# lab-emi/CleanUMamba

Measured on AMD Instinct MI355X. Metric: audio samples/sec/node (train step, E8, 10s@16kHz), higher is better.
Workload: dtype f16

## Files before the change

cleanumamba_amd/csrc/gemm_tn.hip:

```cpp
#include "common.h"

namespace cum {

typedef __attribute__((ext_vector_type(8))) __bf16 bf16x8;
typedef __attribute__((ext_vector_type(4))) __bf16 bf16x4;
typedef __attribute__((ext_vector_type(8))) _Float16 f16x8;
typedef __attribute__((ext_vector_type(4))) _Float16 f16x4;
typedef __attribute__((ext_vector_type(4))) float f32x4;

struct TnParams {
  const void *dZ, *X;
  float *slab;
  float *bslab;
  int64_t ldz, ldx;
  int64_t M;
  int N, K;
  int Np, Kp;
  int rows_per_split, nsplit;
#ifdef CUM_AB
  int skip_store;
#endif
};

constexpr int TN_T = 128;

template <typename T>
struct TnCfg;
template <>
struct TnCfg<__bf16> {
  static constexpr int EPC = 8, BMK = 64;
  static __device__ __forceinline__ int swz(int row) { return 2 * ((row & 3) | (((row >> 3) & 1) << 2)); }
};
template <>
// ... 940 lines not shown
  if (tn_use8(M, N, K, dtype)) {
    *Np = N;
    *Kp = K;
    const int tiles = (N / 256) * (K / 256);
    int64_t want = tiles >= 256 ? 1 : 256 / tiles;
    if (force > 0) want = force;
    const int64_t max_s = (M + 255) / 256;
    if (want > max_s) want = max_s;
    int64_t rows = (M + want - 1) / want;
    rows = (rows + 63) / 64 * 64;
    *rps = (int)rows;
    *S = (int)((M + rows - 1) / rows);
    return;
  }
  *Np = (N + TN_T - 1) / TN_T * TN_T;
  *Kp = (K + TN_T - 1) / TN_T * TN_T;
  const int tiles = (*Np / TN_T) * (*Kp / TN_T);
  const int bmk = is16(dtype) ? 32 : 16;
  const int per_xcd = tiles >= 96 ? 1 : 96 / tiles;
  int64_t want = 8 * per_xcd;
  if (force > 0) want = force;
  const int64_t max_s = (M + 8 * bmk - 1) / (8 * bmk);
  if (want > max_s) want = max_s;
  if (want < 1) want = 1;
  int64_t rows = (M + want - 1) / want;
  rows = (rows + bmk - 1) / bmk * bmk;
  *rps = (int)rows;
  *S = (int)((M + rows - 1) / rows);
  if (*S < 1) *S = 1;
}

static int reduce_chunks(int S) { return S >= 64 ? 16 : 1; }

extern "C" int64_t cum_gemm_tn_workspace_elems(int32_t dtype, int64_t M, int32_t N, int32_t K) {
  int Np, Kp, S, rps;
  tn_plan(M, N, K, dtype, &Np, &Kp, &S, &rps);
  const int64_t C = reduce_chunks(S);
  return (int64_t)S * Np * Kp + (int64_t)S * Np + C * (int64_t)N * K + C * (int64_t)Np;
}

extern "C" int cum_gemm_tn_tile(int32_t dtype, int64_t M, int32_t N, int32_t K) {
  return tn_use8(M, N, K, dtype) ? 256 : tn_use_stream(M, N, K, dtype) ? 384 : TN_T;
}

extern "C" int cum_gemm_tn(int32_t dtype, int64_t M, int32_t N, int32_t K, const void *dZ, int64_t ldz, const void *X,
                           int64_t ldx, float *dW, int64_t ldw, float *db, float *workspace, void *stream) {
  CUM_REQUIRE(dtype_ok(dtype), "gemm_tn: dtype must be CUM_F32, CUM_BF16 or CUM_F16");
  CUM_REQUIRE(dZ && X && dW && workspace && M >= 0 && N > 0 && K > 0, "gemm_tn: bad argument");
  const int epc = is16(dtype) ? 8 : 4;
  CUM_REQUIRE(N % epc == 0 && K % epc == 0 && ldz % epc == 0 && ldx % epc == 0 && ldw % 4 == 0,
              "gemm_tn: N, K and strides must keep 16-byte alignment");
  CUM_REQUIRE(((uintptr_t)dZ & 15) == 0 && ((uintptr_t)X & 15) == 0 && ((uintptr_t)dW & 15) == 0,
              "gemm_tn: pointers must be 16-byte aligned");
  hipStream_t st = (hipStream_t)stream;
  const bool want_bias = db != nullptr;
  if (M == 0) {
    (void)hipMemset2DAsync(dW, sizeof(float) * ldw, 0, sizeof(float) * K, N, st);
    if (db) (void)hipMemsetAsync(db, 0, sizeof(float) * N, st);
    return CUM_OK;
  }
  int Np, Kp, S, rps;
  tn_plan(M, N, K, dtype, &Np, &Kp, &S, &rps);
  TnParams p{};
  p.dZ = dZ; p.X = X; p.ldz = ldz; p.ldx = ldx; p.M = M; p.N = N; p.K = K; p.Np = Np; p.Kp = Kp;
  p.rows_per_split = rps;
  p.nsplit = S;
// ... 6 lines not shown
  if (tn_use8(M, N, K, dtype)) {
    const int items = (N / 256) * (K / 256) * S;
    const dim3 grid8(8 * ((items + 7) / 8)), block8(512);
#ifdef CUM_AB
    if (cum_knob("CUM_TN9", 1) == 0) {
      if (dtype == CUM_BF16) hipLaunchKernelGGL(gemm_tn8_kernel<__bf16>, grid8, block8, 0, st, p);
      else hipLaunchKernelGGL(gemm_tn8_kernel<f16>, grid8, block8, 0, st, p);
    } else
#endif
    if (dtype == CUM_BF16)
      hipLaunchKernelGGL(gemm_tn9_kernel<__bf16>, grid8, block8, 0, st, p);
    else
      hipLaunchKernelGGL(gemm_tn9_kernel<f16>, grid8, block8, 0, st, p);
  } else if (tn_use_stream(M, N, K, dtype)) {
    CUM_REQUIRE((int64_t)rps * (ldz > ldx ? ldz : ldx) + 512 < (int64_t)1 << 31, "gemm_tn: a row split exceeds 2^31 elements");
    const dim3 gs(S), bs(512);
    if (Np == 128) {
      if (dtype == CUM_BF16) hipLaunchKernelGGL((gemm_tn_stream_kernel<__bf16, 128, 256>), gs, bs, 0, st, p);
      else hipLaunchKernelGGL((gemm_tn_stream_kernel<f16, 128, 256>), gs, bs, 0, st, p);
    } else {
      if (dtype == CUM_BF16) hipLaunchKernelGGL((gemm_tn_stream_kernel<__bf16, 256, 128>), gs, bs, 0, st, p);
      else hipLaunchKernelGGL((gemm_tn_stream_kernel<f16, 256, 128>), gs, bs, 0, st, p);
    }
  } else if (dtype == CUM_BF16)
    hipLaunchKernelGGL(gemm_tn_kernel<__bf16>, grid, block, 0, st, p);
  else if (dtype == CUM_F16)
    hipLaunchKernelGGL(gemm_tn_kernel<f16>, grid, block, 0, st, p);
  else
    hipLaunchKernelGGL(gemm_tn_kernel<float>, grid, block, 0, st, p);
  CUM_CHECK_LAUNCH();
#ifdef CUM_AB
  if (cum_knob("CUM_TN_NOREDUCE", 0)) return CUM_OK;
#endif
  const int C = reduce_chunks(S);
  float *part = workspace + (int64_t)S * Np * Kp + (int64_t)S * Np;
  float *bpart = part + (int64_t)C * N * K;
  const int cols4 = K / 4, bc4 = N / 4;
  const int gx = (int)(((int64_t)N * cols4 + 63) / 64), bx = want_bias ? (bc4 + 63) / 64 : 0;
  if (C == 1) {
    const ReduceJob w{p.slab, dW, (int64_t)Np * Kp, 0, ldw, Kp, N, cols4};
    const ReduceJob bj{p.bslab, db, (int64_t)Np, 0, N, Np, 1, bc4};
    hipLaunchKernelGGL(tn_reduce_kernel, dim3(gx + bx, 1), dim3(256), 0, st, w, bj, gx, S);
  } else {
    const ReduceJob w1{p.slab, part, (int64_t)Np * Kp, (int64_t)N * K, (int64_t)K, Kp, N, cols4};
    const ReduceJob b1{p.bslab, bpart, (int64_t)Np, (int64_t)Np, (int64_t)Np, Np, 1, bc4};
    hipLaunchKernelGGL(tn_reduce_kernel, dim3(gx + bx, C), dim3(256), 0, st, w1, b1, gx, S);
    const ReduceJob w2{part, dW, (int64_t)N * K, 0, ldw, K, N, cols4};
    const ReduceJob b2{bpart, db, (int64_t)Np, 0, N, Np, 1, bc4};
    hipLaunchKernelGGL(tn_reduce_kernel, dim3(gx + bx, 1), dim3(256), 0, st, w2, b2, gx, C);
  }
  CUM_CHECK_LAUNCH();
  return CUM_OK;
}
```

cleanumamba_amd/hip.py:

```python
import ctypes
import os

import torch

_HERE = os.path.dirname(os.path.abspath(__file__))
LIB_PATH = os.environ.get("CUM_LIB") or os.path.join(_HERE, "libcleanumamba_hip.so")

c_i32, c_i64, c_f32p, c_vp = ctypes.c_int32, ctypes.c_int64, ctypes.c_void_p, ctypes.c_void_p


class ScanShape(ctypes.Structure):
    _fields_ = [("batch", c_i32), ("dim", c_i32), ("dstate", c_i32), ("len", c_i32),
                ("u_sb", c_i64), ("u_sd", c_i64), ("u_sl", c_i64),
                ("dt_sb", c_i64), ("dt_sd", c_i64), ("dt_sl", c_i64),
                ("z_sb", c_i64), ("z_sd", c_i64), ("z_sl", c_i64),
                ("o_sb", c_i64), ("o_sd", c_i64), ("o_sl", c_i64),
                ("B_sb", c_i64), ("B_sn", c_i64), ("B_sl", c_i64),
                ("C_sb", c_i64), ("C_sn", c_i64), ("C_sl", c_i64),
                ("delta_softplus", c_i32), ("io_dtype", c_i32)]


class ScanGradStrides(ctypes.Structure):
    _fields_ = [("du_sb", c_i64), ("du_sd", c_i64), ("du_sl", c_i64),
                ("dd_sb", c_i64), ("dd_sd", c_i64), ("dd_sl", c_i64),
# ... 78 lines not shown
    "cum_stft_loss_fwd": (c_i32, [_P, _P, c_i64, c_i64, c_i32, c_i64, _P, _P, _P]),
    "cum_stft_loss_bwd": (c_i32, [_P, _P, c_i64, c_i64, c_i32, c_i64, _P, _P, _P, _P, _P]),
    "cum_stft_fold": (c_i32, [_P, c_i64, c_i64, c_i32, c_i32, c_i32, _P, c_i64, _P, c_i64, c_i32, _P]),
    "cum_gather": (c_i32, [c_i32, _P, _P, c_i64, c_i32, _P, _P]),
    "cum_pack2d": (c_i32, [_P, _P, _P, c_i32, _P, c_i32, _P, _P]),
    "cum_add_layernorm_fwd": (c_i32, [c_i32, c_i32, c_i64, c_i32, c_i32, _P, c_i64, c_i64, _P, _P, _P, ctypes.c_float,
                                      _P, _P, _P, _P, _P]),
    "cum_add_layernorm_bwd_workspace_elems": (c_i64, [c_i32]),
    "cum_add_layernorm_bwd": (c_i32, [c_i32, c_i32, c_i64, c_i32] + [_P] * 12),
    "cum_small_linear": (c_i32, [c_i32, c_i32, c_i32, _P, c_i64, _P, _P, _P, c_i64, _P]),
    "cum_mamba_step_supported": (c_i32, [c_i32] * 5),
    "cum_mamba_step": (c_i32, [c_i32] * 6 + [ctypes.c_float] + [_P] * 20),
    "cum_stream_window_update": (c_i32, [c_i32, c_i32, c_i32, c_i32, c_i32, _P, _P, c_i64, c_i64, c_i32, _P, _P, c_i64, _P]),
    "cum_stream_tail_rows": (c_i32, [c_i32, c_i32, c_i32, c_i32, _P, c_i64, c_i32, _P, c_i64, _P]),
    "cum_stream_overlap_add": (c_i32, [c_i32, c_i32, c_i32, c_i32, c_i32, _P, c_i64, _P, _P, _P, c_i64, _P, c_i64, c_i32, _P]),
    "cum_stream_hop_plan_ints": (c_i32, []),
    "cum_stream_hop_max_lds_bytes": (c_i32, []),
    "cum_stream_hop": (c_i32, [_P, _P, _P, c_i64, c_i32, _P, c_i64, _P, c_i64, c_i32, c_i32, _P]),
    "cum_stream_hop_slots": (c_i32, [_P, _P, _P, c_i64, c_i32, _P, _P, c_i32, _P, c_i64, _P, c_i64, c_i32, _P]),
    "cum_stream_pool_stage": (c_i32, [_P, c_i64, c_i32, _P, _P, c_i32, _P, c_i64, _P, c_i64, _P]),
    "cum_fft_plan_create": (c_i32, [c_i32, c_i32, c_i64, ctypes.POINTER(ctypes.c_void_p), ctypes.POINTER(c_i64)]),
    "cum_fft_plan_destroy": (c_i32, [_P]),
    "cum_fft_exec": (c_i32, [_P, _P, _P, c_i32, _P, _P]),
    "cum_stft_fused_supported": (c_i32, [c_i32]),
    "cum_stft_fused_workspace_elems": (c_i64, [c_i64, c_i64]),
    "cum_stft_fused_fwd": (c_i32, [_P, _P, c_i64, c_i64, c_i64, c_i64, c_i32, c_i32, c_i32, _P, _P, c_i64, c_i64, _P, _P, _P]),
    "cum_stft_fused_bwd": (c_i32, [_P, _P, c_i64, c_i64, c_i64, c_i64, c_i32, c_i32, c_i32, _P, _P, c_i64, c_i64, _P, _P, _P,
                                   _P, _P]),
    "cum_stft_loss_fwd_packed": (c_i32, [_P, _P, c_i64, c_i64, c_i32, c_i64, _P, _P, _P, _P]),
    "cum_stft_loss_bwd_packed": (c_i32, [_P, _P, c_i64, c_i64, c_i32, c_i64, _P, _P, _P, _P, _P, _P]),
    "cum_enc0_fwd": (c_i32, [c_i32, c_i64, c_i32, c_i32, _P, _P, _P, _P, _P, _P, c_i64, _P, _P]),
    "cum_ench_fwd": (c_i32, [c_i32, c_i64, c_i32, c_i32, _P, c_i64, _P, _P, _P, _P, _P, c_i64, _P, _P, c_i64, _P, _P]),
    "cum_dech_fwd": (c_i32, [c_i32, c_i64, c_i32, c_i32, _P, c_i64, _P, _P, _P, _P, _P, _P, c_i64, _P, _P, c_i64, _P, _P]),
    "cum_enc0_bwd_workgroups": (c_i32, [c_i64]),
    "cum_enc0_bwd_workspace_elems": (c_i64, [c_i64]),
    "cum_enc0_bwd": (c_i32, [c_i32, c_i64, c_i32, c_i32, _P, _P, _P, _P, _P, _P, _P, _P, _P]),
    "cum_dec7_fwd": (c_i32, [c_i32, c_i64, c_i32, c_i32, _P, _P, _P, _P, _P, _P, c_i64, _P]),
    "cum_dec7_bwd_workgroups": (c_i32, [c_i64]),
    "cum_dec7_bwd_workspace_elems": (c_i64, [c_i64]),
    "cum_dec7_bwd": (c_i32, [c_i32, c_i64, c_i32, c_i32, _P, _P, _P, _P, _P, _P, _P, _P, c_i64, _P, _P, _P, _P]),
    "cum_lp_loss_parts": (c_i32, [c_i64]),
    "cum_lp_loss_fwd": (c_i32, [c_i32, _P, _P, c_i64, _P, _P, _P]),
    "cum_lp_loss_bwd": (c_i32, [c_i32, _P, _P, c_i64, _P, _P, _P]),
    "cum_clip_std_parts": (c_i32, [c_i64]),
    "cum_clip_std": (c_i32, [_P, c_i32, c_i64, c_i64, ctypes.c_float, _P, _P, _P]),
    "cum_frame_rows": (c_i32, [c_i32, _P, c_i32, c_i64, c_i64, c_i64, c_i64, _P, c_i32, _P, _P]),
    "cum_unframe_rows": (c_i32, [c_i32, _P, c_i32, c_i64, c_i64, _P, _P, _P]),
    "cum_optim_state_elems": (c_i32, []),
    "cum_optim_sumsq_parts": (c_i32, [c_i64]),
    "cum_optim_sumsq": (c_i32, [_P, c_i64, _P, _P]),
    "cum_optim_prepare": (c_i32, [_P, _P, c_i32, ctypes.c_float, ctypes.c_double, ctypes.c_double, c_i32, ctypes.c_float,
                                  ctypes.c_float, c_i32, _P]),
    "cum_ssd_chunk": (c_i32, []),
    "cum_ssd_states_elems": (c_i64, [c_i32] * 5),
    "cum_ssd_bwd_workspace_elems": (c_i64, [c_i32] * 5),
    "cum_ssd_fwd": (c_i32, [ctypes.POINTER(SsdShape)] + [_P] * 11),
    "cum_ssd_bwd": (c_i32, [ctypes.POINTER(SsdShape)] + [_P] * 12 + [c_i64, c_i64, _P, c_i64, c_i64] + [_P] * 5),
    "cum_gated_rmsnorm_fwd": (c_i32, [c_i32, c_i64, c_i32, _P, c_i64, _P, c_i64, _P, ctypes.c_float, _P, c_i64, _P, _P]),
    "cum_gated_rmsnorm_bwd_workspace_elems": (c_i64, [c_i32]),
    "cum_gated_rmsnorm_bwd": (c_i32, [c_i32, c_i64, c_i32, _P, c_i64, _P, c_i64, _P, _P, _P, c_i64, _P, c_i64, _P, c_i64,
                                      _P, _P, _P]),
    "cum_ssd_step": (c_i32, [c_i32] * 5 + [ctypes.c_float, _P, c_i64] + [_P] * 9 + [c_i64, _P]),
    "cum_optim_adam": (c_i32, [_P, _P, _P, _P, c_i64, _P, ctypes.c_double, ctypes.c_double, ctypes.c_float, ctypes.c_float,
                               _P]),
    "cum_metrics_frame_count": (c_i64, [c_i64]),
    "cum_metrics_reduce_keep": (c_i64, [c_i64]),
# ... 121 lines not shown
```

cleanumamba_amd/network/convstack.py:

```python
import ctypes
import os

import numpy as np
import torch

from .. import hip


def rup(x, m):
    return (x + m - 1) // m * m


class Geo:

    def __init__(self, B, T, C):
        self.B, self.T, self.C = B, T, C
        self.P = T + 2
        self.Cp = rup(C, 8)
        self.M = B * self.P
        self.slack = 2 + (128 + self.Cp - 1) // self.Cp
        self.R = 1 + self.M + self.slack

    def new(self, dtype, device, zero=False):
        if zero:
# ... 1023 lines not shown
_DECH_FUSED = os.environ.get("CUM_DECH_FUSED", "1") != "0"


def _dech_ok(w1, wt, skip, relu, gi, gg, go, dt):
    return (_DECH_FUSED and _SIGN_MASK and relu and skip is not None and dt in hip.HALF_TYPES
            and tuple(w1.shape) == (256, 128, 1) and tuple(wt.shape) == (128, 64, 4)
            and gi.Cp == 128 and gg.Cp == 128 and go.Cp == 64 and gg.P >= 3)


def _dech_fwd(ubuf, w1, b1, wt, bt, skip, gi, gg, go, save_z):
    dt, dev = ubuf.dtype, ubuf.device
    sh1, sht = tuple(w1.shape), tuple(wt.shape)
    w1p = take(w1, ("glu_fwd", sh1, 256, 128), lambda: lay_glu_fwd(sh1, 256, 128), dt)
    b1p = take(b1, ("glu_vec", 256), lambda: lay_glu_vec(256), torch.float32)
    wtp = take(wt, ("convt_fwd", sht, gg.Cp, go.Cp, 128, 256), lambda: lay_convt_fwd(sht, gg.Cp, go.Cp, 128, 256), dt)

    def bias_layout():
        out = torch.zeros(128, dtype=torch.int64)
        out.view(2, 64)[:, :64] = _ids((64,))
        return out
    btp = take(bt, ("convt_vec", 64, go.Cp, 128), bias_layout, torch.float32)
    ybuf = go.new(dt, dev)
    g = gg.new(dt, dev) if save_z else None
    z = torch.empty(gg.M, 128, dtype=dt, device=dev) if save_z else None
    act = torch.empty(go.R * go.Cp // 4, dtype=torch.uint8, device=dev) if save_z else None
    with torch.cuda.device(dev):
        hip.check(hip.lib().cum_dech_fwd(
            hip.dtype_code(dt), gg.M, gg.P, gg.T, hip.ptr(ubuf), gi.R, hip.ptr(w1p), hip.ptr(b1p), hip.ptr(wtp),
            hip.ptr(btp), hip.ptr(skip[1:]), hip.ptr(g), gg.tail, hip.ptr(z), hip.ptr(ybuf[1:]), go.tail,
            hip.ptr(act[go.Cp // 4:]) if act is not None else None, hip.stream_ptr()))
    return g, z, ybuf, act


def _enc0_bwd(dz, xbuf, w1, b1, w2, gm, go, slot_w1, slot_w2):
    dt, dev = dz.dtype, dz.device
    wp = _enc0_w2p(w2, gm, dt)
    lib = hip.lib()
    ws = torch.empty(lib.cum_enc0_bwd_workspace_elems(go.M), dtype=torch.float32, device=dev)
    (a1, o1), (a2, o2) = slot_w1, slot_w2
    with torch.cuda.device(dev):
        hip.check(lib.cum_enc0_bwd(hip.dtype_code(dt), go.M, go.P, go.T, hip.ptr(dz), hip.ptr(xbuf), hip.ptr(w1.detach()),
                                   hip.ptr(b1.detach()), hip.ptr(wp), ctypes.c_void_p(a2.data_ptr() + 4 * o2),
                                   ctypes.c_void_p(a1.data_ptr() + 4 * o1), hip.ptr(ws), hip.stream_ptr()))


_DEC7_FUSED = os.environ.get("CUM_DEC7_FUSED", "1") != "0"


def _dec7_ok(w1, wt, gi, gg, go, dt):
    return (_DEC7_FUSED and dt in hip.HALF_TYPES and tuple(w1.shape) == (128, 64, 1) and tuple(wt.shape) == (64, 1, 4)
            and gi.C == 64 and gg.C == 64 and go.C == 1 and go.Cp == 8 and gi.P >= 32 and w1.dtype == torch.float32
            and wt.dtype == torch.float32)


def _dec7_fwd(ubuf, w1, b1, wt, bt, gi, go):
    dt, dev = ubuf.dtype, ubuf.device
    wp = _enc0_w2p(w1, gi, dt)
    bp = take(b1, ("glu_vec", w1.shape[0]), lambda: lay_glu_vec(w1.shape[0]), torch.float32)
    ybuf = go.new(dt, dev)
    with torch.cuda.device(dev):
        hip.check(hip.lib().cum_dec7_fwd(hip.dtype_code(dt), gi.M, gi.P, gi.T, hip.ptr(ubuf), hip.ptr(wp), hip.ptr(bp),
                                         hip.ptr(wt.detach()), hip.ptr(bt.detach()), hip.ptr(ybuf), go.tail, hip.stream_ptr()))
    return ybuf


def _dec7_bwd(dy, ubuf, mask_bits, w1, b1, wt, gi, slot_w1, slot_wt):
# ... 58 lines not shown
        def parts(lo, hi):
            out = []
            for i in range(lo, hi):
                gi, gm, _ = geos[i]
                sh1, sh2 = shapes[4 * i], shapes[4 * i + 2]
                G32 = 2 * zs[i].shape[1]
                out.append(arena.dw_index(2 * i, _invert(lay_conv_fwd(sh1, gi.Cp, gm.Cp, 4 * gi.Cp), sh1)))
                out.append(arena.db_index(2 * i, torch.arange(1, sh1[0] + 1, dtype=torch.int64)))
                out.append(arena.dw_index(2 * i + 1, _invert(lay_glu_fwd(sh2, G32, gm.Cp), sh2)))
                out.append(arena.db_index(2 * i + 1, _invert(lay_glu_vec(sh2[0]), (sh2[0],))))
            return out
        key = ("enc", tuple(shapes), tuple((g[0].Cp, g[1].Cp) for g in geos), tuple(z.shape[1] for z in zs))

        def deliver(lo, hi):
            grads[4 * lo:4 * hi] = arena.deliver((key, lo, hi), params[4 * lo:4 * hi], shapes[4 * lo:4 * hi],
                                                 lambda: parts(lo, hi))
        cut = E - 3 if E > 3 else 0
        sink = grad_sink(params) if cut > 0 else None
        early = sink is not None and getattr(sink[0], "early_announce", False)
        for i in reversed(range(E)):
            gi, gm, go = geos[i]
            w1, b1, w2, b2 = params[4 * i:4 * i + 4]
            if dz is None:
                if dys[i] is None:
                    raise RuntimeError("EncoderStack: the deepest output must be used")
                dz = _glu_bwd(zs[i], bufs[i + 1], dys[i].contiguous(), go)
            G32 = dz.shape[1]
            y1 = y1s[i]
            if y1 is None:
                if not ctx.needs_input_grad[0]:
                    _enc0_bwd(dz, bufs[0], w1, b1, w2, gm, go, arena.out(0), arena.out(1))
                    break
                y1 = _conv_relu_fwd(bufs[0], w1, b1, gi, gm)
            _glu_wgrad(dz, y1, gm, go.M, arena.out(2 * i + 1))
            wt = _glu_dgrad_weights(w2, gm, G32, dt)
            dzc = gm.new(dt, dev)
            if bits[i] is not None:
                gemm(dz, 0, G32, wt, None, dzc, gm.Cp, gm.Cp, gm.M, gm.P, gm.T, hip.EPI_MASK, gm.Cp,
                     res=bits[i][gm.Cp // 4:], r_off=0, ldr=gm.Cp, geo=gm, mask_bits=True)
            else:
                gemm(dz, 0, G32, wt, None, dzc, gm.Cp, gm.Cp, gm.M, gm.P, gm.T, hip.EPI_MASK, gm.Cp,
                     res=y1, r_off=gm.Cp, ldr=gm.Cp, geo=gm)
            sh = tuple(w1.shape)
            wgrad(dzc, gm.Cp, gm.Cp, gm.Cp, bufs[i], gi.Cp, 2 * gi.Cp, 4 * gi.Cp, gm.M, out=arena.out(2 * i))
            dz = None
            if early and i == cut:
                deliver(cut, E)
            if i == 0 and not ctx.needs_input_grad[0]:
                break
            Nd, Kd = rup(2 * gi.Cp, 16), rup(2 * gm.Cp, bk_of(dt))
            wd = take(w1, ("conv_dgrad", sh, gi.Cp, gm.Cp, Nd, Kd), lambda: lay_conv_dgrad(sh, gi.Cp, gm.Cp, Nd, Kd), dt)
            ext = None if i == 0 or dys[i - 1] is None else dys[i - 1].contiguous()
            if i > 0 and gi.Cp % 16 == 0:
                dz = torch.empty(gi.M, 2 * gi.Cp, dtype=dt, device=dev)
                gemm(dzc, 0, gm.Cp, wd, None, dz, 0, 4 * gi.Cp, gm.M, gm.P, gm.T + 1, hip.EPI_GLU_BWD, 2 * gi.Cp,
                     res=ext, r_off=gi.Cp, ldr=2 * gi.Cp, aux=zs[i - 1], x_off=0, ldz=2 * gi.Cp,
                     aux2=bufs[i], y_off=gi.Cp, ldy=2 * gi.Cp, gate_only=True)
                continue
            dx = gi.new(dt, dev)
            gemm(dzc, 0, gm.Cp, wd, None, dx, gi.Cp, 2 * gi.Cp, gm.M, gm.P, gm.T + 1, hip.EPI_BIAS, 2 * gi.Cp, geo=gi)
            if i == 0:
                dx0 = dx
            else:
                dz = _glu_bwd(zs[i - 1], bufs[i], dx if ext is None else dx + ext, gi)
        deliver(0, cut if early else E)
        return (dx0, None, None, *grads)


def _convt_bias_grad(bt, dbp, Cp, C, dtype):
    sink = grad_sink([bt]) if (bt.is_leaf and bt.dtype == torch.float32) else None
    if sink is not None:
        flat, idx, offs = sink
        torch.add(dbp[:C], dbp[Cp:Cp + C], out=flat.grad[offs[0]:offs[0] + C])
        flat.wrote(idx)
        return None
# ... 122 lines not shown
```

include/cleanumamba_hip.h:

```cpp
#ifndef CLEANUMAMBA_HIP_H
#define CLEANUMAMBA_HIP_H

#include <stdint.h>

#ifdef __cplusplus
extern "C" {
#endif

#define CUM_OK 0
#define CUM_EINVAL (-1)
#define CUM_ELAUNCH (-2)
#define CUM_EWORKSPACE (-3)

#define CUM_ABI_VERSION 16

int cum_abi_version(void);
const char *cum_last_error(void);

int cum_scan_chunk(void);

#define CUM_SCAN_SOFTPLUS 1
#define CUM_SCAN_A_IS_LOG 2
typedef struct {
  int32_t batch, dim, dstate, len;
// ... 183 lines not shown
int cum_stream_overlap_add(int32_t dtype, int32_t streams, int32_t L2, int32_t Cp, int32_t C, const void *y,
                           int64_t y_pitch, void *tail, const float *bias, const void *skip, int64_t skip_pitch,
                           void *out, int64_t out_pitch, int32_t relu, void *stream);

int cum_stream_hop_plan_ints(void);
int cum_stream_hop_max_lds_bytes(void);
int cum_stream_hop(const void *plan, const float *weights, float *state, int64_t state_stride, int32_t streams,
                   const float *in, int64_t in_stride, float *out, int64_t out_stride, int32_t n_hops,
                   int32_t lds_bytes, void *stream);

int cum_stream_hop_slots(const void *plan, const float *weights, float *state, int64_t state_stride, int32_t capacity,
                         const int32_t *items_host, const int32_t *items, int32_t n_items, const float *in,
                         int64_t in_stride, float *out, int64_t out_stride, int32_t lds_bytes, void *stream);
int cum_stream_pool_stage(float *hist, int64_t hist_stride, int32_t capacity, const int32_t *recs_host,
                          const int32_t *recs, int32_t n_recs, const float *x, int64_t x_stride, float *stage,
                          int64_t stage_stride, void *stream);

int cum_enc0_fwd(int32_t dtype, int64_t M, int32_t pitch, int32_t valid, const void *xin, const float *w1,
                 const float *b1, const void *w2p, const float *b2p, void *out, int64_t zero_tail, void *gate,
                 void *stream);
int32_t cum_enc0_bwd_workgroups(int64_t M);
int64_t cum_enc0_bwd_workspace_elems(int64_t M);
int cum_enc0_bwd(int32_t dtype, int64_t M, int32_t pitch, int32_t valid, const void *dZ, const void *xin,
                 const float *w1, const float *b1, const void *w2p, float *slot_w2, float *slot_w1, float *workspace,
                 void *stream);

int cum_ench_fwd(int32_t dtype, int64_t M, int32_t pitch, int32_t valid, const void *xin, int64_t x_rows,
                 const void *w1p, const float *b1p, const void *w2p, const float *b2p, void *y1, int64_t y1_tail,
                 void *bits, void *out, int64_t out_tail, void *gate, void *stream);

int cum_dech_fwd(int32_t dtype, int64_t M, int32_t pitch, int32_t valid, const void *u, int64_t u_rows,
                 const void *w1p, const float *b1p, const void *wtp, const float *btp, const void *skip, void *g,
                 int64_t g_tail, void *gate, void *out, int64_t out_tail, void *bits, void *stream);

int cum_dec7_fwd(int32_t dtype, int64_t M, int32_t pitch, int32_t valid, const void *u, const void *w1p, const float *b1p,
                 const float *wt, const float *bt, void *out, int64_t zero_tail, void *stream);
int32_t cum_dec7_bwd_workgroups(int64_t M);
int64_t cum_dec7_bwd_workspace_elems(int64_t M);
int cum_dec7_bwd(int32_t dtype, int64_t M, int32_t pitch, int32_t valid, const void *dY, const void *u, const void *mask,
                 const void *w1p, const float *b1p, const float *wt, void *dU, void *dpre, int64_t zero_tail,
                 float *slot_w1, float *slot_wt, float *workspace, void *stream);

int32_t cum_lp_loss_parts(int64_t n);
int cum_lp_loss_fwd(int32_t p, const float *y, const float *c, int64_t n, float *partials, float *out, void *stream);
int cum_lp_loss_bwd(int32_t p, const float *y, const float *c, int64_t n, const float *gout, float *dy, void *stream);

int32_t cum_clip_std_parts(int64_t len);
int cum_clip_std(const float *x, int32_t rows, int64_t len, int64_t stride, float eps, float *partials, float *out,
                 void *stream);

int cum_frame_rows(int32_t dtype, const float *x, int32_t batch, int64_t len, int64_t stride, int64_t T,
                   int64_t total_rows, const float *scale, int32_t invert, void *out, void *stream);
int cum_unframe_rows(int32_t dtype, const void *rows, int32_t batch, int64_t len, int64_t T, const float *scale,
                     float *y, void *stream);

int32_t cum_optim_state_elems(void);
int32_t cum_optim_sumsq_parts(int64_t n);
int cum_optim_sumsq(const float *g, int64_t n, float *partials, void *stream);
int cum_optim_prepare(float *state, const float *partials, int32_t nparts, float max_norm, double beta1, double beta2,
                      int32_t use_scaler, float growth, float backoff, int32_t growth_interval, void *stream);
int cum_optim_adam(float *p, const float *g, float *m, float *v, int64_t n, const float *state, double beta1,
                   double beta2, float eps, float weight_decay, void *stream);

typedef struct {
  int32_t batch, len, nheads, headdim, dstate;
  int64_t x_sb, x_sl, dt_sb, dt_sl, B_sb, B_sl, C_sb, C_sl, y_sb, y_sl;
// ... 80 lines not shown
```

Before: 130.8 million.

## Fuse GLU weight-grad and masked data-grad GEMMs into one pointwise pair backward kernel

Adds a HIP kernel that streams dZ and X tiles through LDS once and computes both the weight gradient (TN GEMM, with bias sum into per-split slabs) and the masked data gradient (dZ times W with sign-bit mask and valid-time zeroing) in the same pass. The slab reduction is factored out of gemm_tn so the new kernel can reuse it. The encoder backward path uses the new kernel for the 256x128 pointwise layer when mask bits exist. The goal is to avoid reading dZ twice and to save a launch, in exchange for a specialized, shape-restricted kernel with inline-asm wait counts.

```diff
diff --git a/cleanumamba_amd/csrc/gemm_tn.h b/cleanumamba_amd/csrc/gemm_tn.h
--- /dev/null
+++ b/cleanumamba_amd/csrc/gemm_tn.h
@@ -0,0 +1,10 @@
+#pragma once
+#include "common.h"
+
+namespace cum {
+
+int tn_reduce_chunks(int S);
+void tn_reduce_slabs(const float *slab, const float *bslab, float *part, int S, int N, int K, int Np, int Kp, float *dW,
+                     int64_t ldw, float *db, hipStream_t st);
+
+}
diff --git a/cleanumamba_amd/csrc/gemm_tn.hip b/cleanumamba_amd/csrc/gemm_tn.hip
--- a/cleanumamba_amd/csrc/gemm_tn.hip
+++ b/cleanumamba_amd/csrc/gemm_tn.hip
@@ -1,4 +1,5 @@
 #include "common.h"
+#include "gemm_tn.h"
 
 namespace cum {
 
@@ -1005,6 +1006,30 @@
 
 static int reduce_chunks(int S) { return S >= 64 ? 16 : 1; }
 
+namespace cum {
+int tn_reduce_chunks(int S) { return reduce_chunks(S); }
+void tn_reduce_slabs(const float *slab, const float *bslab, float *part, int S, int N, int K, int Np, int Kp, float *dW,
+                     int64_t ldw, float *db, hipStream_t st) {
+  const bool want_bias = bslab != nullptr;
+  const int C = reduce_chunks(S);
+  float *bpart = part + (int64_t)C * N * K;
+  const int cols4 = K / 4, bc4 = N / 4;
+  const int gx = (int)(((int64_t)N * cols4 + 63) / 64), bx = want_bias ? (bc4 + 63) / 64 : 0;
+  if (C == 1) {
+    const ReduceJob w{slab, dW, (int64_t)Np * Kp, 0, ldw, Kp, N, cols4};
+    const ReduceJob bj{bslab, db, (int64_t)Np, 0, N, Np, 1, bc4};
+    hipLaunchKernelGGL(tn_reduce_kernel, dim3(gx + bx, 1), dim3(256), 0, st, w, bj, gx, S);
+  } else {
+    const ReduceJob w1{slab, part, (int64_t)Np * Kp, (int64_t)N * K, (int64_t)K, Kp, N, cols4};
+    const ReduceJob b1{bslab, bpart, (int64_t)Np, (int64_t)Np, (int64_t)Np, Np, 1, bc4};
+    hipLaunchKernelGGL(tn_reduce_kernel, dim3(gx + bx, C), dim3(256), 0, st, w1, b1, gx, S);
+    const ReduceJob w2{part, dW, (int64_t)N * K, 0, ldw, K, N, cols4};
+    const ReduceJob b2{bpart, db, (int64_t)Np, 0, N, Np, 1, bc4};
+    hipLaunchKernelGGL(tn_reduce_kernel, dim3(gx + bx, 1), dim3(256), 0, st, w2, b2, gx, C);
+  }
+}
+}
+
 extern "C" int64_t cum_gemm_tn_workspace_elems(int32_t dtype, int64_t M, int32_t N, int32_t K) {
   int Np, Kp, S, rps;
   tn_plan(M, N, K, dtype, &Np, &Kp, &S, &rps);
@@ -1077,23 +1102,7 @@
 #ifdef CUM_AB
   if (cum_knob("CUM_TN_NOREDUCE", 0)) return CUM_OK;
 #endif
-  const int C = reduce_chunks(S);
-  float *part = workspace + (int64_t)S * Np * Kp + (int64_t)S * Np;
-  float *bpart = part + (int64_t)C * N * K;
-  const int cols4 = K / 4, bc4 = N / 4;
-  const int gx = (int)(((int64_t)N * cols4 + 63) / 64), bx = want_bias ? (bc4 + 63) / 64 : 0;
-  if (C == 1) {
-    const ReduceJob w{p.slab, dW, (int64_t)Np * Kp, 0, ldw, Kp, N, cols4};
-    const ReduceJob bj{p.bslab, db, (int64_t)Np, 0, N, Np, 1, bc4};
-    hipLaunchKernelGGL(tn_reduce_kernel, dim3(gx + bx, 1), dim3(256), 0, st, w, bj, gx, S);
-  } else {
-    const ReduceJob w1{p.slab, part, (int64_t)Np * Kp, (int64_t)N * K, (int64_t)K, Kp, N, cols4};
-    const ReduceJob b1{p.bslab, bpart, (int64_t)Np, (int64_t)Np, (int64_t)Np, Np, 1, bc4};
-    hipLaunchKernelGGL(tn_reduce_kernel, dim3(gx + bx, C), dim3(256), 0, st, w1, b1, gx, S);
-    const ReduceJob w2{part, dW, (int64_t)N * K, 0, ldw, K, N, cols4};
-    const ReduceJob b2{bpart, db, (int64_t)Np, 0, N, Np, 1, bc4};
-    hipLaunchKernelGGL(tn_reduce_kernel, dim3(gx + bx, 1), dim3(256), 0, st, w2, b2, gx, C);
-  }
+  tn_reduce_slabs(p.slab, p.bslab, workspace + (int64_t)S * Np * Kp + (int64_t)S * Np, S, N, K, Np, Kp, dW, ldw, db, st);
   CUM_CHECK_LAUNCH();
   return CUM_OK;
 }
diff --git a/cleanumamba_amd/csrc/pair_bwd.hip b/cleanumamba_amd/csrc/pair_bwd.hip
--- /dev/null
+++ b/cleanumamba_amd/csrc/pair_bwd.hip
@@ -0,0 +1,388 @@
+#include "common.h"
+#include "gemm_tn.h"
+
+namespace cum {
+
+typedef __attribute__((ext_vector_type(8))) __bf16 pw_bf16x8;
+typedef __attribute__((ext_vector_type(8))) _Float16 pw_f16x8;
+typedef __attribute__((ext_vector_type(4))) float pw_f32x4;
+typedef __attribute__((ext_vector_type(2))) unsigned pw_u32x2;
+typedef __attribute__((ext_vector_type(4))) unsigned pw_u32x4;
+
+struct PairParams {
+  const void *dZ, *X, *W;
+  const unsigned char *bits;
+  void *out, *aux;
+  float *slab, *bslab;
+  int64_t M, out_tail;
+  int rows_per_split, nsplit;
+  unsigned pitch, valid;
+};
+
+__device__ __forceinline__ int pw_swz(int row) { return 2 * ((row & 3) | (((row >> 3) & 1) << 2)); }
+
+template <typename T>
+__device__ __forceinline__ pw_f32x4 pw_mfma(pw_u32x4 a, pw_u32x4 b, pw_f32x4 c) {
+  if constexpr (__is_same(T, f16))
+    return __builtin_amdgcn_mfma_f32_16x16x32_f16(__builtin_bit_cast(pw_f16x8, a), __builtin_bit_cast(pw_f16x8, b), c, 0, 0, 0);
+  else
+    return __builtin_amdgcn_mfma_f32_16x16x32_bf16(__builtin_bit_cast(pw_bf16x8, a), __builtin_bit_cast(pw_bf16x8, b), c, 0, 0, 0);
+}
+
+template <typename T>
+__device__ __forceinline__ unsigned pw_pack2(float a, float b) {
+  typedef T V2 __attribute__((ext_vector_type(2)));
+  V2 v = {(T)a, (T)b};
+  return __builtin_bit_cast(unsigned, v);
+}
+
+template <typename T, bool AUX>
+__global__ __launch_bounds__(512) void pw_pair_bwd_kernel(const PairParams p) {
+  static_assert(sizeof(T) == 2, "16-bit element types only");
+  constexpr int NT = 256, KT = 128;
+  constexpr int EPC = 8, BMK = 64, NST = 3;
+  constexpr int CZ = NT / EPC, CX = KT / EPC;
+  constexpr int ZCH = BMK * CZ, XCH = BMK * CX;
+  constexpr int BCH = BMK * (KT / 4) / 16;
+  constexpr int NZ = ZCH / 512, NX = XCH / 512;
+  constexpr int NDMA = NZ + NX + 1;
+  constexpr int NSTORE = AUX ? 8 : 4;
+  constexpr int STG = ZCH + XCH + BCH;
+  constexpr int WN = NT / 64;
+  __shared__ uint4 lds[NST * STG];
+
+  const int tid = threadIdx.x, lane = tid & 63;
+  const int wave = uniform(tid >> 6);
+  const int wn = wave % WN, wk = wave / WN;
+  const int g = lane >> 4, r = lane & 15;
+  const int sp = blockIdx.x;
+  const int64_t m_begin = (int64_t)sp * p.rows_per_split;
+  int64_t m_end = m_begin + p.rows_per_split;
+  m_end = m_end < p.M ? m_end : p.M;
+  const int rows = (int)(m_end - m_begin);
+  const T *dZ = static_cast<const T *>(p.dZ) + m_begin * NT;
+  const T *X = static_cast<const T *>(p.X) + m_begin * KT;
+  const unsigned char *bits = p.bits ? p.bits + m_begin * (KT / 4) : nullptr;
+  T *out = static_cast<T *>(p.out) + m_begin * KT;
+  T *aux = AUX ? static_cast<T *>(p.aux) + m_begin * KT : nullptr;
+
+  typedef __attribute__((address_space(3))) void *lds_ptr;
+  typedef const __attribute__((address_space(1))) void *glb_ptr;
+
+  pw_u32x4 wf[8];
+  {
+    const T *W = static_cast<const T *>(p.W) + (16 * wave + r) * NT + 8 * g;
+#pragma unroll
+    for (int kb = 0; kb < 8; ++kb) wf[kb] = *reinterpret_cast<const pw_u32x4 *>(W + 32 * kb);
+    asm volatile("s_waitcnt vmcnt(0)"
+                 : "+v"(wf[0]), "+v"(wf[1]), "+v"(wf[2]), "+v"(wf[3]), "+v"(wf[4]), "+v"(wf[5]), "+v"(wf[6]), "+v"(wf[7])
+                 : : "memory");
+  }
+
+  int zrow[NZ], zoff[NZ], xrow[NX], xoff[NX];
+#pragma unroll
+  for (int i = 0; i < NZ; ++i) {
+    const int pos = i * 512 + tid;
+    zrow[i] = pos / CZ;
+    zoff[i] = ((pos % CZ) ^ pw_swz(zrow[i])) * EPC;
+  }
+#pragma unroll
+  for (int i = 0; i < NX; ++i) {
+    const int pos = i * 512 + tid;
+    xrow[i] = pos / CX;
+    xoff[i] = ((pos % CX) ^ pw_swz(xrow[i])) * EPC;
+  }
+  const int brow = tid >> 3, boff = (tid & 7) * 4;
+  auto issue = [&](int s, int buf) {
+    uint4 *st = lds + buf * STG;
+#pragma unroll
+    for (int i = 0; i < NZ; ++i) {
+      int m = s * BMK + zrow[i];
+      m = m < rows ? m : rows - 1;
+      __builtin_amdgcn_global_load_lds((glb_ptr)(dZ + (m * NT + zoff[i])), (lds_ptr)(&st[i * 512 + wave * 64]), 16, 0, 0);
+    }
+#pragma unroll
+    for (int i = 0; i < NX; ++i) {
+      int m = s * BMK + xrow[i];
+      m = m < rows ? m : rows - 1;
+      __builtin_amdgcn_global_load_lds((glb_ptr)(X + (m * KT + xoff[i])), (lds_ptr)(&st[ZCH + i * 512 + wave * 64]), 16, 0, 0);
+    }
+    {
+      int m = s * BMK + brow;
+      m = m < rows ? m : rows - 1;
+      const unsigned char *src = bits ? bits + (m * (KT / 4) + boff) : reinterpret_cast<const unsigned char *>(dZ + m * NT) + boff;
+      __builtin_amdgcn_global_load_lds((glb_ptr)src, (lds_ptr)(&st[ZCH + XCH + wave * 16]), 4, 0, 0);
+    }
+  };
+
+  constexpr int BROWS = 512 / CZ;
+  const int bc = tid % CZ;
+  float bsum[EPC];
+#pragma unroll
+  for (int e = 0; e < EPC; ++e) bsum[e] = 0.f;
+
+  pw_f32x4 acc[4][4];
+#pragma unroll
+  for (int i = 0; i < 4; ++i)
+#pragma unroll
+    for (int j = 0; j < 4; ++j) acc[i][j] = pw_f32x4{0.f, 0.f, 0.f, 0.f};
+
+  const unsigned lds0 = (unsigned)(uintptr_t)(lds_ptr)lds;
+  const int q = r >> 2, pp = r & 3;
+  const int r0 = 8 * g + q, s0 = pw_swz(r0);
+  unsigned ax[4], az[4], ab[BMK / BROWS], ad[4];
+#pragma unroll
+  for (int i = 0; i < 4; ++i) {
+    ax[i] = (unsigned)((ZCH + r0 * CX + ((wk * 8 + 2 * i) ^ s0)) * 16 + pp * 8);
+    az[i] = (unsigned)((r0 * CZ + ((wn * 8 + 2 * i) ^ s0)) * 16 + pp * 8);
+    ad[i] = (unsigned)((r * CZ + ((4 * i + g) ^ pw_swz(r))) * 16);
+  }
+#pragma unroll
+  for (int i = 0; i < BMK / BROWS; ++i) {
+    const int row = tid / CZ + BROWS * i;
+    ab[i] = (unsigned)((row * CZ + (bc ^ pw_swz(row))) * 16);
+  }
+  const unsigned am = (unsigned)((ZCH + XCH) * 16 + r * (KT / 4) + 4 * wave + g);
+#define CUM_TR(dst, addr, off) asm volatile("ds_read_b64_tr_b16 %0, %1 offset:%2" : "=v"(dst) : "v"(addr), "n"(off) : "memory")
+#define CUM_RD128(dst, addr, off) asm volatile("ds_read_b128 %0, %1 offset:%2" : "=v"(dst) : "v"(addr), "n"(off) : "memory")
+
+  unsigned t0 = (unsigned)(m_begin % p.pitch);
+  const int nsteps = (rows + BMK - 1) / BMK;
+  issue(0, 0);
+  if (nsteps > 1) issue(1, 1);
+  int buf = 0;
+  for (int s = 0; s < nsteps; ++s) {
+    if (s + 1 < nsteps) {
+      if (s == 0) asm volatile("s_waitcnt vmcnt(%0)" ::"n"(NDMA) : "memory");
+      else asm volatile("s_waitcnt vmcnt(%0)" ::"n"(NDMA + NSTORE) : "memory");
+    } else {
+      asm volatile("s_waitcnt vmcnt(0)" ::: "memory");
+    }
+    const bool full = (s + 1) * BMK <= rows;
+    if (!full) {
+      uint4 *st = lds + buf * STG;
+#pragma unroll
+      for (int i = 0; i < NZ; ++i)
+        if (s * BMK + zrow[i] >= rows) st[i * 512 + tid] = make_uint4(0, 0, 0, 0);
+#pragma unroll
+      for (int i = 0; i < NX; ++i)
+        if (s * BMK + xrow[i] >= rows) st[ZCH + i * 512 + tid] = make_uint4(0, 0, 0, 0);
+      asm volatile("s_waitcnt lgkmcnt(0)" ::: "memory");
+    }
+    asm volatile("s_barrier" ::: "memory");
+    if (s + 2 < nsteps) issue(s + 2, buf == 0 ? 2 : buf - 1);
+    const unsigned sb = lds0 + (unsigned)(buf * STG * 16);
+
+    {
+      pw_u32x2 xl[2][4], xh[2][4], zl[2][4], zh[2][4];
+      pw_u32x4 bv[BMK / BROWS];
+#pragma unroll
+      for (int i = 0; i < 4; ++i) {
+        CUM_TR(xl[0][i], sb + ax[i], 0);
+        CUM_TR(xh[0][i], sb + ax[i], 4 * CX * 16);
+        CUM_TR(zl[0][i], sb + az[i], 0);
+        CUM_TR(zh[0][i], sb + az[i], 4 * CZ * 16);
+      }
+#pragma unroll
+      for (int i = 0; i < BMK / BROWS; ++i) CUM_RD128(bv[i], sb + ab[i], 0);
+#pragma unroll
+      for (int kk = 0; kk < 2; ++kk) {
+#define CUM_TR_WAIT(n)                                                                                              \
+  asm volatile("s_waitcnt lgkmcnt(%16)"                                                                            \
+               : "+v"(xl[kk][0]), "+v"(xl[kk][1]), "+v"(xl[kk][2]), "+v"(xl[kk][3]), "+v"(xh[kk][0]), "+v"(xh[kk][1]), \
+                 "+v"(xh[kk][2]), "+v"(xh[kk][3]), "+v"(zl[kk][0]), "+v"(zl[kk][1]), "+v"(zl[kk][2]), "+v"(zl[kk][3]), \
+                 "+v"(zh[kk][0]), "+v"(zh[kk][1]), "+v"(zh[kk][2]), "+v"(zh[kk][3])                                    \
+               : "n"(n) : "memory")
+        __builtin_amdgcn_sched_barrier(0);
+        if (kk == 0) CUM_TR_WAIT(BMK / BROWS);
+        else CUM_TR_WAIT(0);
+#undef CUM_TR_WAIT
+        if (kk == 0) {
+#pragma unroll
+          for (int i = 0; i < 4; ++i) {
+            CUM_TR(xl[1][i], sb + ax[i], 32 * CX * 16);
+            CUM_TR(xh[1][i], sb + ax[i], 36 * CX * 16);
+            CUM_TR(zl[1][i], sb + az[i], 32 * CZ * 16);
+            CUM_TR(zh[1][i], sb + az[i], 36 * CZ * 16);
+          }
+          __builtin_amdgcn_sched_barrier(0);
+        }
+        pw_u32x4 xf[4], zf[4];
+#pragma unroll
+        for (int i = 0; i < 4; ++i) {
+          xf[i] = __builtin_shufflevector(xl[kk][i], xh[kk][i], 0, 1, 2, 3);
+          zf[i] = __builtin_shufflevector(zl[kk][i], zh[kk][i], 0, 1, 2, 3);
+        }
+#pragma unroll
+        for (int ki = 0; ki < 4; ++ki)
+#pragma unroll
+          for (int ni = 0; ni < 4; ++ni) acc[ki][ni] = pw_mfma<T>(xf[ki], zf[ni], acc[ki][ni]);
+        if (kk == 0) {
+          __builtin_amdgcn_sched_barrier(0);
+          asm volatile("s_waitcnt lgkmcnt(15)" : "+v"(bv[0]), "+v"(bv[1]), "+v"(bv[2]), "+v"(bv[3]) : : "memory");
+#pragma unroll
+          for (int i = 0; i < BMK / BROWS; ++i) {
+            if constexpr (__is_same(T, f16)) {
+              const pw_f16x8 h = __builtin_bit_cast(pw_f16x8, bv[i]);
+#pragma unroll
+              for (int e = 0; e < 8; ++e) bsum[e] += (float)h[e];
+            } else {
+              const pw_bf16x8 h = __builtin_bit_cast(pw_bf16x8, bv[i]);
+#pragma unroll
+              for (int e = 0; e < 8; ++e) bsum[e] += (float)h[e];
+            }
+          }
+        }
+      }
+    }
+
+    {
+      __builtin_amdgcn_sched_barrier(0);
+      pw_u32x4 f[2][4];
+      unsigned mb[4];
+#pragma unroll
+      for (int rb = 0; rb < 4; ++rb)
+        asm volatile("ds_read_u8 %0, %1 offset:%2" : "=v"(mb[rb]) : "v"(sb + am), "n"(rb * 16 * (KT / 4)) : "memory");
+#pragma unroll
+      for (int h = 0; h < 2; ++h)
+#pragma unroll
+        for (int i = 0; i < 4; ++i) CUM_RD128(f[h][i], sb + ad[i], h * 256);
+#pragma unroll
+      for (int rb = 0; rb < 4; ++rb) {
+        pw_f32x4 d = pw_f32x4{0.f, 0.f, 0.f, 0.f};
+#pragma unroll
+        for (int h = 0; h < 2; ++h) {
+          __builtin_amdgcn_sched_barrier(0);
+          if (rb == 3 && h == 1)
+            asm volatile("s_waitcnt lgkmcnt(0)" : "+v"(f[h][0]), "+v"(f[h][1]), "+v"(f[h][2]), "+v"(f[h][3]),
+                         "+v"(mb[0]), "+v"(mb[1]), "+v"(mb[2]), "+v"(mb[3]) : : "memory");
+          else
+            asm volatile("s_waitcnt lgkmcnt(4)" : "+v"(f[h][0]), "+v"(f[h][1]), "+v"(f[h][2]), "+v"(f[h][3]),
+                         "+v"(mb[0]), "+v"(mb[1]), "+v"(mb[2]), "+v"(mb[3]) : : "memory");
+#pragma unroll
+          for (int i = 0; i < 4; ++i) d = pw_mfma<T>(wf[4 * h + i], f[h][i], d);
+          __builtin_amdgcn_sched_barrier(0);
+          if (rb < 3) {
+#pragma unroll
+            for (int i = 0; i < 4; ++i) {
+              if (rb == 0) CUM_RD128(f[h][i], sb + ad[i], 1 * 16 * CZ * 16 + h * 256);
+              else if (rb == 1) CUM_RD128(f[h][i], sb + ad[i], 2 * 16 * CZ * 16 + h * 256);
+              else CUM_RD128(f[h][i], sb + ad[i], 3 * 16 * CZ * 16 + h * 256);
+            }
+          }
+        }
+        const int row = s * BMK + rb * 16 + r;
+        unsigned tt = t0 + (unsigned)(rb * 16 + r);
+        tt = tt >= p.pitch ? tt - p.pitch : tt;
+        const bool real = tt < p.valid;
+        const unsigned nib = bits ? mb[rb] : 0xFu;
+        float u[4], v[4];
+#pragma unroll
+        for (int j = 0; j < 4; ++j) {
+          u[j] = real ? d[j] : 0.f;
+          v[j] = ((nib >> j) & 1u) ? u[j] : 0.f;
+        }
+        const pw_u32x2 vo = pw_u32x2{pw_pack2<T>(v[0], v[1]), pw_pack2<T>(v[2], v[3])};
+        const pw_u32x2 uo = pw_u32x2{pw_pack2<T>(u[0], u[1]), pw_pack2<T>(u[2], u[3])};
+        const int eo = row * KT + 16 * wave + 4 * g;
+        if (full || row < rows) {
+          asm volatile("global_store_dwordx2 %0, %1, off" : : "v"(out + eo), "v"(vo) : "memory");
+          if constexpr (AUX) asm volatile("global_store_dwordx2 %0, %1, off" : : "v"(aux + eo), "v"(uo) : "memory");
+        }
+      }
+    }
+    t0 += BMK;
+    t0 = t0 >= p.pitch ? t0 - p.pitch : t0;
+    buf = buf == NST - 1 ? 0 : buf + 1;
+  }
+#undef CUM_TR
+#undef CUM_RD128
+
+  float *slab = p.slab + (int64_t)sp * NT * KT;
+#pragma unroll
+  for (int ni = 0; ni < 4; ++ni) {
+    const int n = wn * 64 + ni * 16 + r;
+#pragma unroll
+    for (int ki = 0; ki < 4; ++ki) {
+      const int k = wk * 64 + ki * 16 + 4 * g;
+      *reinterpret_cast<float4 *>(slab + (int64_t)n * KT + k) =
+          make_float4(acc[ki][ni][0], acc[ki][ni][1], acc[ki][ni][2], acc[ki][ni][3]);
+    }
+  }
+  {
+    __syncthreads();
+    float *red = reinterpret_cast<float *>(lds);
+    const int tr = tid / CZ;
+#pragma unroll
+    for (int e = 0; e < EPC; ++e) red[tr * NT + bc * EPC + e] = bsum[e];
+    __syncthreads();
+    if (tid < NT) {
+      float sum = 0.f;
+      for (int j = 0; j < 512 / CZ; ++j) sum += red[j * NT + tid];
+      p.bslab[(int64_t)sp * NT + tid] = sum;
+    }
+  }
+  if (sp == 0 && tid < KT / 8) {
+    reinterpret_cast<uint4 *>(static_cast<T *>(p.out) - KT)[tid] = make_uint4(0, 0, 0, 0);
+    if constexpr (AUX) reinterpret_cast<uint4 *>(static_cast<T *>(p.aux) - KT)[tid] = make_uint4(0, 0, 0, 0);
+  }
+  if (sp == p.nsplit - 1) {
+    for (int64_t i = tid; i < p.out_tail / 8; i += 512) {
+      reinterpret_cast<uint4 *>(static_cast<T *>(p.out) + p.M * KT)[i] = make_uint4(0, 0, 0, 0);
+      if constexpr (AUX) reinterpret_cast<uint4 *>(static_cast<T *>(p.aux) + p.M * KT)[i] = make_uint4(0, 0, 0, 0);
+    }
+  }
+}
+
+}
+
+using namespace cum;
+
+static void pw_plan(int64_t M, int *S, int *rps) {
+  int64_t rows = (M + 255) / 256;
+  rows = (rows + 63) / 64 * 64;
+  *rps = (int)rows;
+  *S = (int)((M + rows - 1) / rows);
+}
+
+extern "C" int64_t cum_pw_pair_bwd_workspace_elems(int64_t M) {
+  if (M <= 0) return 1;
+  int S, rps;
+  pw_plan(M, &S, &rps);
+  const int64_t C = tn_reduce_chunks(S);
+  return (int64_t)S * 256 * 128 + (int64_t)S * 256 + C * (256 * 128 + 256);
+}
+
+extern "C" int cum_pw_pair_bwd(int32_t dtype, int64_t M, int32_t pitch, int32_t valid, const void *dZ, const void *X,
+                               const void *wt, const void *bits, void *out, void *aux, int64_t out_tail, float *slot,
+                               float *workspace, void *stream) {
+  CUM_REQUIRE(is16(dtype), "pw_pair_bwd: dtype must be CUM_BF16 or CUM_F16");
+  CUM_REQUIRE(dZ && X && wt && out && slot && workspace && M > 0, "pw_pair_bwd: bad argument");
+  CUM_REQUIRE(pitch >= 64 && valid >= 0 && valid <= pitch, "pw_pair_bwd: pitch must be >= 64, valid within it");
+  CUM_REQUIRE(out_tail >= 0 && out_tail % 8 == 0, "pw_pair_bwd: out_tail must be a multiple of 8 elements");
+  CUM_REQUIRE(((uintptr_t)dZ & 15) == 0 && ((uintptr_t)X & 15) == 0 && ((uintptr_t)wt & 15) == 0 && ((uintptr_t)out & 15) == 0 &&
+                  ((uintptr_t)aux & 15) == 0 && ((uintptr_t)bits & 3) == 0 && ((uintptr_t)slot & 15) == 0,
+              "pw_pair_bwd: pointers must be 16-byte aligned (sign nibbles: 4-byte)");
+  int S, rps;
+  pw_plan(M, &S, &rps);
+  CUM_REQUIRE((int64_t)rps * 256 + 512 < (int64_t)1 << 31, "pw_pair_bwd: a row split exceeds 2^31 elements");
+  PairParams p{};
+  p.dZ = dZ; p.X = X; p.W = wt; p.bits = static_cast<const unsigned char *>(bits); p.out = out; p.aux = aux;
+  p.M = M; p.out_tail = out_tail; p.rows_per_split = rps; p.nsplit = S;
+  p.pitch = (unsigned)pitch; p.valid = (unsigned)valid;
+  p.slab = workspace;
+  p.bslab = workspace + (int64_t)S * 256 * 128;
+  hipStream_t st = (hipStream_t)stream;
+  const dim3 gs(S), bs(512);
+  if (aux) {
+    if (dtype == CUM_BF16) hipLaunchKernelGGL((pw_pair_bwd_kernel<__bf16, true>), gs, bs, 0, st, p);
+    else hipLaunchKernelGGL((pw_pair_bwd_kernel<f16, true>), gs, bs, 0, st, p);
+  } else {
+    if (dtype == CUM_BF16) hipLaunchKernelGGL((pw_pair_bwd_kernel<__bf16, false>), gs, bs, 0, st, p);
+    else hipLaunchKernelGGL((pw_pair_bwd_kernel<f16, false>), gs, bs, 0, st, p);
+  }
+  CUM_CHECK_LAUNCH();
+  tn_reduce_slabs(p.slab, p.bslab, p.bslab + (int64_t)S * 256, S, 256, 128, 256, 128, slot, 128, slot + 256 * 128, st);
+  CUM_CHECK_LAUNCH();
+  return CUM_OK;
+}
diff --git a/cleanumamba_amd/hip.py b/cleanumamba_amd/hip.py
--- a/cleanumamba_amd/hip.py
+++ b/cleanumamba_amd/hip.py
@@ -134,6 +134,8 @@
     "cum_enc0_fwd": (c_i32, [c_i32, c_i64, c_i32, c_i32, _P, _P, _P, _P, _P, _P, c_i64, _P, _P]),
     "cum_ench_fwd": (c_i32, [c_i32, c_i64, c_i32, c_i32, _P, c_i64, _P, _P, _P, _P, _P, c_i64, _P, _P, c_i64, _P, _P]),
     "cum_dech_fwd": (c_i32, [c_i32, c_i64, c_i32, c_i32, _P, c_i64, _P, _P, _P, _P, _P, _P, c_i64, _P, _P, c_i64, _P, _P]),
+    "cum_pw_pair_bwd_workspace_elems": (c_i64, [c_i64]),
+    "cum_pw_pair_bwd": (c_i32, [c_i32, c_i64, c_i32, c_i32, _P, _P, _P, _P, _P, _P, c_i64, _P, _P, _P]),
     "cum_enc0_bwd_workgroups": (c_i32, [c_i64]),
     "cum_enc0_bwd_workspace_elems": (c_i64, [c_i64]),
     "cum_enc0_bwd": (c_i32, [c_i32, c_i64, c_i32, c_i32, _P, _P, _P, _P, _P, _P, _P, _P, _P]),
diff --git a/cleanumamba_amd/network/convstack.py b/cleanumamba_amd/network/convstack.py
--- a/cleanumamba_amd/network/convstack.py
+++ b/cleanumamba_amd/network/convstack.py
@@ -1079,6 +1079,29 @@
     return g, z, ybuf, act
 
 
+_PW_PAIR = True
+
+
+def _pw_pair_ok(w, g, G32, dt):
+    return (_PW_PAIR and dt in hip.HALF_TYPES and tuple(w.shape) == (256, 128, 1) and G32 == 256 and g.Cp == 128
+            and g.P >= 64 and g.M > 0)
+
+
+def _pw_pair_bwd(dz, xbuf, w, g, gate, slot, want_aux):
+    dt, dev = dz.dtype, dz.device
+    wt = _glu_dgrad_weights(w, g, 256, dt)
+    lib = hip.lib()
+    out = g.new(dt, dev)
+    aux = g.new(dt, dev) if want_aux else None
+    ws = torch.empty(lib.cum_pw_pair_bwd_workspace_elems(g.M), dtype=torch.float32, device=dev)
+    a, o = slot
+    with torch.cuda.device(dev):
+        hip.check(lib.cum_pw_pair_bwd(hip.dtype_code(dt), g.M, g.P, g.T, hip.ptr(dz), hip.ptr(xbuf[1:]), hip.ptr(wt),
+                                      hip.ptr(gate), hip.ptr(out[1:]), hip.ptr(aux[1:]) if want_aux else None, g.tail,
+                                      ctypes.c_void_p(a.data_ptr() + 4 * o), hip.ptr(ws), hip.stream_ptr()))
+    return out, aux
+
+
 def _enc0_bwd(dz, xbuf, w1, b1, w2, gm, go, slot_w1, slot_w2):
     dt, dev = dz.dtype, dz.device
     wp = _enc0_w2p(w2, gm, dt)
@@ -1203,15 +1226,18 @@
                     _enc0_bwd(dz, bufs[0], w1, b1, w2, gm, go, arena.out(0), arena.out(1))
                     break
                 y1 = _conv_relu_fwd(bufs[0], w1, b1, gi, gm)
-            _glu_wgrad(dz, y1, gm, go.M, arena.out(2 * i + 1))
-            wt = _glu_dgrad_weights(w2, gm, G32, dt)
-            dzc = gm.new(dt, dev)
-            if bits[i] is not None:
-                gemm(dz, 0, G32, wt, None, dzc, gm.Cp, gm.Cp, gm.M, gm.P, gm.T, hip.EPI_MASK, gm.Cp,
-                     res=bits[i][gm.Cp // 4:], r_off=0, ldr=gm.Cp, geo=gm, mask_bits=True)
+            if bits[i] is not None and go.M == gm.M and _pw_pair_ok(w2, gm, G32, dt):
+                dzc, _ = _pw_pair_bwd(dz, y1, w2, gm, bits[i][gm.Cp // 4:], arena.out(2 * i + 1), False)
             else:
-                gemm(dz, 0, G32, wt, None, dzc, gm.Cp, gm.Cp, gm.M, gm.P, gm.T, hip.EPI_MASK, gm.Cp,
-                     res=y1, r_off=gm.Cp, ldr=gm.Cp, geo=gm)
+                _glu_wgrad(dz, y1, gm, go.M, arena.out(2 * i + 1))
+                wt = _glu_dgrad_weights(w2, gm, G32, dt)
+                dzc = gm.new(dt, dev)
+                if bits[i] is not None:
+                    gemm(dz, 0, G32, wt, None, dzc, gm.Cp, gm.Cp, gm.M, gm.P, gm.T, hip.EPI_MASK, gm.Cp,
+                         res=bits[i][gm.Cp // 4:], r_off=0, ldr=gm.Cp, geo=gm, mask_bits=True)
+                else:
+                    gemm(dz, 0, G32, wt, None, dzc, gm.Cp, gm.Cp, gm.M, gm.P, gm.T, hip.EPI_MASK, gm.Cp,
+                         res=y1, r_off=gm.Cp, ldr=gm.Cp, geo=gm)
             sh = tuple(w1.shape)
             wgrad(dzc, gm.Cp, gm.Cp, gm.Cp, bufs[i], gi.Cp, 2 * gi.Cp, 4 * gi.Cp, gm.M, out=arena.out(2 * i))
             dz = None
diff --git a/include/cleanumamba_hip.h b/include/cleanumamba_hip.h
--- a/include/cleanumamba_hip.h
+++ b/include/cleanumamba_hip.h
@@ -239,6 +239,10 @@
 int cum_dech_fwd(int32_t dtype, int64_t M, int32_t pitch, int32_t valid, const void *u, int64_t u_rows,
                  const void *w1p, const float *b1p, const void *wtp, const float *btp, const void *skip, void *g,
                  int64_t g_tail, void *gate, void *out, int64_t out_tail, void *bits, void *stream);
+
+int64_t cum_pw_pair_bwd_workspace_elems(int64_t M);
+int cum_pw_pair_bwd(int32_t dtype, int64_t M, int32_t pitch, int32_t valid, const void *dZ, const void *X, const void *wt,
+                    const void *bits, void *out, void *aux, int64_t out_tail, float *slot, float *workspace, void *stream);
 
 int cum_dec7_fwd(int32_t dtype, int64_t M, int32_t pitch, int32_t valid, const void *u, const void *w1p, const float *b1p,
                  const float *wt, const float *bt, void *out, int64_t zero_tail, void *stream);
```

Result: no change. 131.1 million, median of 6 (+0.2%).
